# pnnl/nmrfit

Hardware: NVIDIA B200
Metric: voigt_objective_evals_per_s (higher is better)
Workload: dtype f64

## Files before the change

### include/nmrfit_b200.h

```cpp
#ifndef NMRFIT_B200_H
#define NMRFIT_B200_H

#ifdef __cplusplus
extern "C" {
#endif

#define NMRFIT_ABI_VERSION 2

#define NMRFIT_OK 0
#define NMRFIT_ERR_ARG (-1)
#define NMRFIT_ERR_CUDA (-2)
#define NMRFIT_ERR_STATE (-3)
#define NMRFIT_ERR_NOMEM (-4)

#define NMRFIT_FP64 0
#define NMRFIT_FP32 1

#define NMRFIT_ALGO_AUTO 0
#define NMRFIT_ALGO_GENERAL 1
#define NMRFIT_ALGO_UNIFORM 2

#define NMRFIT_REAL_ONLY 0
#define NMRFIT_IM_REFERENCE 1
#define NMRFIT_IM_SUM 2
// ... 31 lines not shown
#define NMRFIT_REFINE_MAX_ITER 3
#define NMRFIT_REFINE_NONFINITE 4

int nmrfit_ctx_refine(nmrfit_ctx* ctx, double* x_inout, const double* lb, const double* ub, int max_iter, double xtol,
                      double* f_out, int* passes_out, int* accepted_out, int* status_out, void* stream);

int nmrfit_ctx_set_algorithm(nmrfit_ctx* ctx, int algorithm);
int nmrfit_ctx_get_algorithm(nmrfit_ctx* ctx, int fit_im, int* algorithm);

int nmrfit_ctx_set_tuning(nmrfit_ctx* ctx, int threads, int points_per_thread, int exp_table_bits,
                          int particles_per_cta);
int nmrfit_ctx_get_tuning(nmrfit_ctx* ctx, int n_particles, int* threads, int* points_per_thread, int* exp_table_bits,
                          int* particles_per_cta, int* n_point_tiles);
int nmrfit_ctx_set_variant(nmrfit_ctx* ctx, int variant, int stages, int occupancy);
int nmrfit_ctx_get_variant(nmrfit_ctx* ctx, int n_particles, int* variant, int* stages);
int nmrfit_ctx_set_far_cells(nmrfit_ctx* ctx, int cells);

#define NMRFIT_FUSED_AUTO 0
#define NMRFIT_FUSED_OFF 1
#define NMRFIT_FUSED_REQUIRE 2
int nmrfit_ctx_set_fused(nmrfit_ctx* ctx, int mode);
int nmrfit_ctx_fused_launches(nmrfit_ctx* ctx, long long* launches);
int nmrfit_ctx_fused_timing(nmrfit_ctx* ctx, int enable, long long* cycles);

int nmrfit_ctx_profile(nmrfit_ctx* ctx, int enable);
int nmrfit_ctx_profile_read(nmrfit_ctx* ctx, double* total_ms, long long* launches);
int nmrfit_ctx_profile_read_split(nmrfit_ctx* ctx, double* prepare_ms, double* evaluate_ms, long long* launches);

int nmrfit_objective_batch(nmrfit_ctx* ctx, const double* x_dev, int n_particles, int fit_im, double* f_dev,
                           void* stream);
// ... 94 lines not shown
```

### nmrfit_b200/_cabi.py

```python
import ctypes
import os

import numpy as np

_HERE = os.path.dirname(os.path.abspath(__file__))
LIB_PATH = os.environ.get('NMRFIT_B200_LIB') or os.path.join(_HERE, 'csrc', 'libnmrfit_b200.so')

OK = 0
FP64, FP32 = 0, 1
REAL_ONLY, IM_REFERENCE, IM_SUM = 0, 1, 2
ALGO_AUTO, ALGO_GENERAL, ALGO_UNIFORM = 0, 1, 2
FUSED_AUTO, FUSED_OFF, FUSED_REQUIRE = 0, 1, 2
RUNNING, STOP_MINFUNC, STOP_MINSTEP, STOP_MAXITER, STOP_PEER_LOST = 0, 1, 2, 3, 4
REFINE_CONVERGED, REFINE_STALLED, REFINE_MAX_ITER, REFINE_NONFINITE = 1, 2, 3, 4

c_double_p = ctypes.POINTER(ctypes.c_double)
c_int_p = ctypes.POINTER(ctypes.c_int)


class NmrfitError(RuntimeError):

    def __init__(self, code, message):
        super().__init__('libnmrfit_b200 error %d: %s' % (code, message))
        self.code = code
# ... 15 lines not shown
    'nmrfit_device_count': (_i, [c_int_p]),
    'nmrfit_ctx_create': (_i, [ctypes.POINTER(_vp), _i, _i, _i, _i, _i]),
    'nmrfit_ctx_destroy': (None, [_vp]),
    'nmrfit_ctx_set_spectrum': (_i, [_vp, _i, _vp, _vp, _vp, _vp]),
    'nmrfit_ctx_set_spectra': (_i, [_vp, _i, _i, _vp, _vp, _vp, _vp]),
    'nmrfit_ctx_compute_weights': (_i, [_vp, _vp, _vp, _i, _i, _d, _vp, _vp]),
    'nmrfit_ctx_normal_equations': (_i, [_vp, _vp, _vp, _vp, _vp, _vp, _vp]),
    'nmrfit_normal_eq_plan': (_i, [_i, _i, c_int_p]),
    'nmrfit_ctx_refine': (_i, [_vp, _vp, _vp, _vp, _i, _d, _vp, _vp, _vp, _vp, _vp]),
    'nmrfit_ctx_set_algorithm': (_i, [_vp, _i]),
    'nmrfit_ctx_get_algorithm': (_i, [_vp, _i, c_int_p]),
    'nmrfit_ctx_set_tuning': (_i, [_vp, _i, _i, _i, _i]),
    'nmrfit_ctx_get_tuning': (_i, [_vp, _i, c_int_p, c_int_p, c_int_p, c_int_p, c_int_p]),
    'nmrfit_ctx_set_variant': (_i, [_vp, _i, _i, _i]),
    'nmrfit_ctx_get_variant': (_i, [_vp, _i, c_int_p, c_int_p]),
    'nmrfit_ctx_set_far_cells': (_i, [_vp, _i]),
    'nmrfit_ctx_set_fused': (_i, [_vp, _i]),
    'nmrfit_ctx_fused_launches': (_i, [_vp, ctypes.POINTER(ctypes.c_longlong)]),
    'nmrfit_ctx_fused_timing': (_i, [_vp, _i, _vp]),
    'nmrfit_ctx_profile': (_i, [_vp, _i]),
    'nmrfit_ctx_profile_read': (_i, [_vp, c_double_p, ctypes.POINTER(ctypes.c_longlong)]),
    'nmrfit_ctx_profile_read_split': (_i, [_vp, c_double_p, c_double_p, ctypes.POINTER(ctypes.c_longlong)]),
    'nmrfit_objective_batch': (_i, [_vp, _vp, _i, _i, _vp, _vp]),
    'nmrfit_objective_batch_host': (_i, [_vp, _vp, _i, _i, _vp]),
    'nmrfit_ctx_mt19937_shape': (_i, [_vp, ctypes.c_longlong]),
    'nmrfit_ctx_mt19937': (_i, [_vp, _vp, c_int_p, ctypes.c_longlong, ctypes.POINTER(_vp), ctypes.POINTER(_vp), _vp]),
    'nmrfit_pso_begin': (_i, [_vp, _vp, _vp, ctypes.POINTER(PsoOpts), _vp, _vp, _vp]),
    'nmrfit_pso_advance': (_i, [_vp, _vp, _vp, _vp]),
    'nmrfit_pso_step': (_i, [_vp, _vp, _vp, _vp]),
    'nmrfit_pso_peer_export': (_i, [_vp, _i, _i, _vp, ctypes.POINTER(_vp)]),
# ... 203 lines not shown
    def set_algorithm(self, algorithm=ALGO_AUTO):
        check(lib().nmrfit_ctx_set_algorithm(self._h, int(algorithm)))

    def get_algorithm(self, fit_im=REAL_ONLY):
        a = ctypes.c_int(0)
        check(lib().nmrfit_ctx_get_algorithm(self._h, int(fit_im), ctypes.byref(a)))
        return a.value

    def set_tuning(self, threads=0, points_per_thread=0, exp_table_bits=0, particles_per_cta=0):
        check(lib().nmrfit_ctx_set_tuning(self._h, threads, points_per_thread, exp_table_bits, particles_per_cta))

    def get_tuning(self, n_particles):
        vals = [ctypes.c_int(0) for _ in range(5)]
        check(lib().nmrfit_ctx_get_tuning(self._h, int(n_particles), *[ctypes.byref(v) for v in vals]))
        keys = ('threads', 'points_per_thread', 'exp_table_bits', 'particles_per_cta', 'n_point_tiles')
        return dict(zip(keys, (v.value for v in vals)))

    def set_variant(self, variant=-1, stages=0, occupancy=0):
        check(lib().nmrfit_ctx_set_variant(self._h, int(variant), int(stages), int(occupancy)))

    def set_far_cells(self, cells=0):
        check(lib().nmrfit_ctx_set_far_cells(self._h, int(cells)))

    def get_variant(self, n_particles):
        v, st = ctypes.c_int(0), ctypes.c_int(0)
        check(lib().nmrfit_ctx_get_variant(self._h, int(n_particles), ctypes.byref(v), ctypes.byref(st)))
        return v.value, st.value

    def set_fused(self, mode=FUSED_AUTO):
        check(lib().nmrfit_ctx_set_fused(self._h, int(mode)))

# ... 395 lines not shown
```

### nmrfit_b200/csrc/cabi.cu

```cuda
#include <cuda_runtime.h>
#include <algorithm>
#include <cmath>
#include <atomic>
#include <cstdio>
#include <cstring>
#include <memory>
#include <new>
#include <string>
#include <utility>
#include <vector>
#include "../../include/nmrfit_b200.h"
#include "nmrfit_internal.h"

namespace nmrfit {
std::atomic<long long> g_launches{0};
void count_launches(int n) { g_launches.fetch_add(n, std::memory_order_relaxed); }
}

using namespace nmrfit;

namespace {

thread_local std::string t_error;

// ... 62 lines not shown
}

}

constexpr int kShadowSpectra = 4;

struct nmrfit_ctx {
    int device = 0, B = 0, N = 0, P = 0, D = 0, precision = 0;
    DevBuf<double> spec;
    std::vector<char> spec_set;
    std::vector<std::vector<double>> shadow;
    DevBuf<double> grid_h;
    std::vector<char> uniform;
    int algorithm = NMRFIT_ALGO_AUTO;
    DevBuf<double> partials, x_stage, f_stage;
    DevBuf<double> prep_coef, prep_part, prep_far, prep_anchor;
    DevBuf<unsigned> prep_mask;
    ObjTune user_tune{0, 0, 0, 0, -1, 0, 0};
    bool swarm = false;
    SwarmState sw{};
    int maxiter = 0, kk = 0, generation = 0;
    DevBuf<double> sx, sv, sp, sfx, sfp, sg, sfg, sbx, sbf, slb, sub, srec, rnd_a, rnd_b;
    DevBuf<int> sstop, sit;
    DevBuf<double> frec_f, frec_x;
    DevBuf<unsigned> fbarrier;
    DevBuf<int> ferror;
    DevBuf<unsigned> mt_state;
    DevBuf<unsigned> mt_words;
    long long mt_elems = 0;
    DevBuf<double> mt_a[2], mt_b[2];
    DevBuf<unsigned> mt_state2, mt_words2;
// ... 63 lines not shown
    grid[0] = h;
    grid[1] = 2.220446049250313e-16 * big;
    return uni;
}

bool use_uniform(const nmrfit_ctx* c, int fit_im) {
    if (c->algorithm == NMRFIT_ALGO_GENERAL) return false;
    if (fit_im == NMRFIT_IM_SUM || (fit_im == NMRFIT_IM_REFERENCE && c->precision != NMRFIT_FP64)) return false;
    for (char u : c->uniform)
        if (!u) return false;
    return true;
}

int ctx_cells(const nmrfit_ctx* c, int r) { return c->far_cells ? c->far_cells : far_cells_per_region(c->N, r); }

ObjTune pick_tune(const nmrfit_ctx* c, int S, bool uni) {
    ObjTune t;
    if (uni) {
        if (c->N >= 2048) { t.threads = 256; t.r = 8; }
        else { t.threads = 128; t.r = 4; }
    } else {
        if (c->N >= 8192) { t.threads = 256; t.r = 4; }
        else if (c->N >= 1024) { t.threads = 128; t.r = 4; }
        else { t.threads = 128; t.r = 2; }
    }
    t.tb = 6;
    if (c->user_tune.threads) t.threads = c->user_tune.threads;
    if (c->user_tune.r) t.r = c->user_tune.r;
    if (c->user_tune.tb == -1) t.tb = 0;
    else if (c->user_tune.tb > 0) t.tb = c->user_tune.tb;
    int n_tiles = (c->N + t.threads * t.r - 1) / (t.threads * t.r);
    long long ctas1 = (long long)n_tiles * S * c->B;
    int sp = (int)std::max<long long>(1, std::min<long long>(16, ctas1 / (148 * 4)));
    sp = std::min(sp, std::max(1, S));
    if (c->user_tune.sp > 0) sp = std::min(c->user_tune.sp, std::max(1, S));
    t.sp = sp;
    t.variant = 0;
    t.stages = 0;
    t.occ = 3;
    const long long particle_tiles = (long long)((c->N + t.threads * t.r - 1) / (t.threads * t.r)) * S * c->B;
    const bool enough = particle_tiles >= 8192 || c->user_tune.variant == 1;
    if (uni && c->precision == NMRFIT_FP64 && c->user_tune.variant != 0 && t.tb == 6 && enough) {
        t.variant = 1;
        t.occ = c->user_tune.occ == 3 ? 3 : 2;
        const size_t budget = t.occ == 2 ? 115712 : 74 * 1024;
        const int cells = ctx_cells(c, t.r), per_warp = t.occ == 2 ? cells : 1;
        auto fit_sp = [&](int stg) {
            t.stages = stg;
            int spg = 0;
            for (int cand = 1; cand <= 16; ++cand) {
                t.sp = cand;
                if (objective_stream_smem_bytes(c->P, t, cells) <= budget && (cand < per_warp || cand % per_warp == 0))
                    spg = cand;
            }
            return spg;
        };
        int stg = c->user_tune.stages > 0 ? c->user_tune.stages : 3;
        int spg = fit_sp(stg);
        if (c->user_tune.stages == 0 && spg < 6) {
            const int spg2 = fit_sp(2);
            if (spg2 > spg) { stg = 2; spg = spg2; }
        }
        t.stages = stg;
        t.sp = std::max(1, spg);
        bool fits = true;
        if (c->user_tune.sp > 0) {
            t.sp = c->user_tune.sp;
            if (objective_stream_smem_bytes(c->P, t, ctx_cells(c, t.r)) > 200 * 1024 && c->user_tune.stages == 0) t.stages = 2;
            fits = objective_stream_smem_bytes(c->P, t, ctx_cells(c, t.r)) <= 200 * 1024;
        }
        if (fits) {
            t.sp = std::min(t.sp, std::max(1, S));
            return t;
        }
        t.variant = 0;
        t.stages = 0;
        t.occ = 3;
    }
    const bool f32 = c->precision == NMRFIT_FP32;
    auto uni_bytes = [&]() { return f32 ? objective_f32_smem_bytes(c->P, t) : objective_uniform_smem_bytes(c->P, t, ctx_cells(c, t.r)); };
    while (t.sp > 1 && (uni ? uni_bytes() : objective_smem_bytes(c->P, t, 2)) > 200 * 1024)
        t.sp /= 2;
    if (uni && c->user_tune.sp <= 0)
        while (t.sp > 4 && uni_bytes() > 74 * 1024) t.sp -= 1;
    return t;
}

int check_ctx(const nmrfit_ctx* c) {
    if (!c) return fail(NMRFIT_ERR_ARG, "ctx is NULL");
    return NMRFIT_OK;
}

// ... 12 lines not shown

struct ObjOut {
    int n_tiles = 0, nsum = 1, nw = 1;
};

int run_objective(nmrfit_ctx* c, const double* x_dev, int S, int fit_im, double* f_dev, cudaStream_t st,
                  const ObjIn& in = {}, ObjOut* out = nullptr) {
    for (int b = 0; b < c->B; ++b)
        if (!c->spec_set[b]) return fail(NMRFIT_ERR_STATE, "spectrum " + std::to_string(b) + " was never set");
    if (fit_im < 0 || fit_im > 2) return fail(NMRFIT_ERR_ARG, "fit_im must be 0, 1 or 2");
    const bool uni = use_uniform(c, fit_im);
    if (c->algorithm == NMRFIT_ALGO_UNIFORM && !uni)
        return fail(NMRFIT_ERR_STATE, "the uniform-axis kernel needs uniformly spaced w in every spectrum and fit_im off");
    if (c->precision == NMRFIT_FP32 && fit_im != NMRFIT_REAL_ONLY)
        return fail(NMRFIT_ERR_ARG, "fit_im is not available in FP32 mode (the Kramers-Kronig term runs in FP64 only)");
    ObjTune t = pick_tune(c, S, uni);
    if (uni && c->precision == NMRFIT_FP32 && t.r == 16) t.r = 8;
    if (uni ? (t.r != 4 && t.r != 8 && t.r != 16) : (t.r != 2 && t.r != 4 && t.r != 8))
        return fail(NMRFIT_ERR_ARG, uni ? "points_per_thread must be 4, 8 or 16 for the uniform-axis kernel"
                                        : "points_per_thread must be 2, 4 or 8 for the general kernel");
    int n_tiles = objective_tiles(c->N, t);
    const size_t part_per = (size_t)n_tiles * 2 * (t.variant == 1 ? t.threads / 32 : 1);
    CK(c->partials.reserve(std::max((size_t)c->B * S, in.slots_total) * part_per));
    ObjArgs a{};
    const int sub = (uni && c->precision == NMRFIT_FP64) ? ctx_cells(c, t.r) : 1;
    if (uni) {
        size_t nc, np, nf, na, nm;
        int pad = 0;
        objective_uniform_prep_sizes(c->N, c->P, t, sub, &nc, &np, &nf, &na, &nm, &pad);
        const size_t slots = std::max((size_t)c->B * S, in.slots_total) + pad;
        CK(c->prep_coef.reserve(slots * nc));
        CK(c->prep_part.reserve(slots * np));
        CK(c->prep_far.reserve(slots * nf));
        CK(c->prep_anchor.reserve(slots * na));
        CK(c->prep_mask.reserve(slots * nm));
        a.prep_coef = c->prep_coef.ptr + in.slot0 * nc; a.prep_part = c->prep_part.ptr + in.slot0 * np;
        a.prep_far = c->prep_far.ptr + in.slot0 * nf; a.prep_anchor = c->prep_anchor.ptr + in.slot0 * na;
        a.prep_mask = c->prep_mask.ptr + in.slot0 * nm;
    }
    a.spec = c->spec.ptr;
    a.x = x_dev;
    a.x_in = in.x_in;
    a.partials = c->partials.ptr + in.slot0 * part_per;
    a.frozen = in.frozen;
    a.grid_h = c->grid_h.ptr;
    a.N = c->N; a.P = c->P; a.S = S; a.kk = fit_im; a.sp = t.sp; a.sub = sub;
    cudaEvent_t ev0 = nullptr, evm = nullptr, ev1 = nullptr;
    if (c->profiling) {
        if (c->prof_used + 3 > c->prof_events.size()) {
            for (int k = 0; k < 3; ++k) {
                cudaEvent_t ev;
                CK(cudaEventCreate(&ev));
                c->prof_events.emplace_back(ev);
// ... 28 lines not shown

int stage(const double* src, size_t n, DevBuf<double>& buf, cudaStream_t st, const double** out) {
    if (!src) { *out = nullptr; return NMRFIT_OK; }
    if (is_device_pointer(src)) { *out = src; return NMRFIT_OK; }
    CK(buf.reserve(n));
    CK(cudaMemcpyAsync(buf.ptr, src, n * sizeof(double), cudaMemcpyHostToDevice, st));
    *out = buf.ptr;
    return NMRFIT_OK;
}

int fused_setup(nmrfit_ctx* c, int n_gen, const double* rp_d, const double* rg_d, FusedArgs* a, FusedPlan* plan) {
    plan->ok = false;
    if (c->fused_mode == NMRFIT_FUSED_OFF) return NMRFIT_OK;
    if (c->precision != NMRFIT_FP64 || c->kk != NMRFIT_REAL_ONLY || !use_uniform(c, NMRFIT_REAL_ONLY)) return NMRFIT_OK;
    const SwarmState& s = c->sw;
    ObjTune t = pick_tune(c, s.S, true);
    *a = FusedArgs{};
    a->s = s;
    a->spec = c->spec.ptr;
    a->grid_h = c->grid_h.ptr;
    a->rp = rp_d;
    a->rg = rg_d;
    a->N = c->N; a->P = c->P;
    a->n_vtiles = objective_tiles(c->N, t);
    a->vw = t.threads / 32;
    a->sub = ctx_cells(c, t.r);
    a->n_gen = n_gen;
    a->gen0 = c->generation + 1;
    a->maxiter = c->maxiter;
    cudaError_t e = swarm_fused_plan(*a, c->D, s.B, s.S, t, c->device, c->fused_mode == NMRFIT_FUSED_REQUIRE, plan);
    if (e != cudaSuccess) return fail_cuda(e, "fused swarm plan");
// ... 360 lines not shown
    c->user_tune.variant = variant;
    c->user_tune.stages = stages;
    c->user_tune.occ = occupancy;
    return NMRFIT_OK;
}

int nmrfit_ctx_set_far_cells(nmrfit_ctx* c, int cells) {
    if (int rc = check_ctx(c)) return rc;
    if (cells != 0 && cells != 1 && cells != 2 && cells != 4) return fail(NMRFIT_ERR_ARG, "cells must be 0 (auto), 1, 2 or 4");
    c->far_cells = cells;
    return NMRFIT_OK;
}

int nmrfit_ctx_get_variant(nmrfit_ctx* c, int S, int* variant, int* stages) {
    if (int rc = check_ctx(c)) return rc;
    ObjTune t = pick_tune(c, S < 1 ? 1 : S, use_uniform(c, NMRFIT_REAL_ONLY));
    if (variant) *variant = t.variant;
    if (stages) *stages = t.stages;
    return NMRFIT_OK;
}

int nmrfit_ctx_get_tuning(nmrfit_ctx* c, int S, int* threads, int* r, int* tb, int* sp, int* n_tiles) {
    if (int rc = check_ctx(c)) return rc;
    ObjTune t = pick_tune(c, S < 1 ? 1 : S, use_uniform(c, NMRFIT_REAL_ONLY));
    if (threads) *threads = t.threads;
    if (r) *r = t.r;
    if (tb) *tb = t.tb;
    if (sp) *sp = t.sp;
    if (n_tiles) *n_tiles = objective_tiles(c->N, t);
    return NMRFIT_OK;
}

int nmrfit_ctx_set_fused(nmrfit_ctx* c, int mode) {
    if (int rc = check_ctx(c)) return rc;
    if (mode != NMRFIT_FUSED_AUTO && mode != NMRFIT_FUSED_OFF && mode != NMRFIT_FUSED_REQUIRE)
        return fail(NMRFIT_ERR_ARG, "mode must be NMRFIT_FUSED_AUTO, _OFF or _REQUIRE");
    c->fused_mode = mode;
    return NMRFIT_OK;
}
// ... 948 lines not shown
```

### nmrfit_b200/csrc/nmrfit_internal.h

```cpp
#pragma once
#include <cuda_runtime.h>
#include <cstddef>
#include <cstdint>

#define NMRFIT_MAX_DEVICES 16

namespace nmrfit {

void count_launches(int n);

struct ObjArgs {
    const double* spec;
    const double* x;
    const double* x_in;
    double* partials;
    const int* frozen;
    const double* grid_h;
    double* prep_coef;
    double* prep_part;
    double* prep_far;
    double* prep_anchor;
    unsigned* prep_mask;
    int n_tiles, nw;
    int N, P, S;
    int kk;
    int sp;
    int tile_major;
    int stages, gpc, occ;
    int sub;
};

__host__ __device__ inline int far_cells_per_region(int N, int R) {
    const int target = N < 8192 ? 64 : (N < 32768 ? 128 : 256);
    int sub = 32 * R / target;
    return sub < 1 ? 1 : (sub > 4 ? 4 : sub);
}

struct ObjTune {
    int threads;
    int r;
    int tb;
    int sp;
    int variant;
    int stages;
    int occ;
};

int objective_tiles(int N, const ObjTune& t);
size_t objective_smem_bytes(int P, const ObjTune& t, int kk);
cudaError_t launch_objective(ObjArgs a, const ObjTune& t, int B, double* f, cudaStream_t st, cudaEvent_t ev0 = nullptr,
                             cudaEvent_t ev1 = nullptr, int* tiles_out = nullptr);

cudaError_t launch_objective_finalize(const double* partials, int n_tiles, int nsum, int N, int S, int B,
                                      const int* frozen, double* f, cudaStream_t st, int nw = 1);

size_t objective_uniform_smem_bytes(int P, const ObjTune& t, int sub = 1);
void objective_uniform_prep_sizes(int N, int P, const ObjTune& t, int sub, size_t* coef, size_t* part, size_t* far,
                                  size_t* anchor, size_t* mask_words, int* pad_particles);
struct SwarmState;
struct MoveArgs;
cudaError_t launch_objective_uniform(ObjArgs a, const ObjTune& t, int B, double* f, cudaStream_t st,
                                     cudaEvent_t ev0 = nullptr, cudaEvent_t ev1 = nullptr, const MoveArgs* mv = nullptr,
                                     int* tiles_out = nullptr, cudaEvent_t evm = nullptr, int* nw_out = nullptr);

cudaError_t launch_objective_prepare(ObjArgs& a, const ObjTune& t, int B, cudaStream_t st, const MoveArgs* mv = nullptr);

size_t objective_stream_smem_bytes(int P, const ObjTune& t, int sub);
cudaError_t launch_objective_stream(const ObjArgs& a, const ObjTune& t, int B, cudaStream_t st);

size_t objective_f32_smem_bytes(int P, const ObjTune& t);
cudaError_t launch_objective_f32(ObjArgs a, const ObjTune& t, int B, double* f, bool uniform, cudaStream_t st,
                                 cudaEvent_t ev0 = nullptr, cudaEvent_t ev1 = nullptr, int* tiles_out = nullptr);

// ... 131 lines not shown
```

### nmrfit_b200/csrc/objective_stream.cu

```cuda
#include <cuda_runtime.h>
#include <algorithm>
#include <cstdint>
#include "nmrfit_internal.h"
#include "nmrfit_math.cuh"
#include "uniform_common.cuh"
#include "uniform_eval.cuh"

namespace nmrfit {

namespace {

template <int TB> struct ExpTabS { static __device__ __forceinline__ const double* src() { return nullptr; } };
template <> struct ExpTabS<6> { static __device__ __forceinline__ const double* src() { return NMRFIT_EXP2_TAB6; } };

struct StreamSmem {
    int tab, uv, wt, wfirst, bars, tickets, slot0, slot, coef, part, far, anchor, mask, mw, total;
    __host__ __device__ StreamSmem(int spg, int stages, int P, int threads, int R, int TB, int sub) {
        const int nw = threads / 32;
        mw = (P + 31) / 32;
        int o = 0;
        tab = o;     o += TB ? (1 << TB) : 0;
        uv = o;      o += threads * R * 2;
        wt = o;      o += threads * R;
        wfirst = o;  o += threads;
        bars = o;    o += stages;
        tickets = o; o += (stages + 1) / 2 * 2;
        if (o & 1) ++o;
        slot0 = o;
        int q = 0;
        coef = q;    q += spg * P * 8;
        part = q;    q += spg * kPartDoubles;
        far = q;     q += spg * nw * sub * kFarPoly;
        anchor = q;  q += spg * nw * 2;
        mask = q;    q += ((spg * nw * mask_words_per_region(P, sub) + 3) / 4) * 2;
        slot = q;
        total = slot0 + stages * slot;
    }
};

__device__ __forceinline__ void fence_proxy_async_smem() { asm volatile("fence.proxy.async.shared::cta;" ::: "memory"); }

template <int THREADS, int R, int TB, int KK, int OCC, int SUB>
__global__ void __launch_bounds__(THREADS, (R <= 8 ? OCC * 256 : 512) / THREADS)
objective_stream_kernel(ObjArgs a) {
    constexpr int NSUM = KK ? 2 : 1;
    constexpr int NW = THREADS / 32;
    constexpr bool MULTI = SUB > 1 && !KK && OCC == 2;
    extern __shared__ __align__(16) double smem[];
    const int b = blockIdx.z;
    if (a.frozen && a.frozen[b]) return;
    const int tid = threadIdx.x, lane = tid & 31, warp = tid >> 5;
    const int P = a.P, N = a.N, D = 4 + 3 * P, SPG = a.sp, ST = a.stages;
    const int n_tiles = a.n_tiles, tile = blockIdx.y, NRP = n_tiles * NW;
    const StreamSmem L(SPG, ST, P, THREADS, R, TB, SUB);
    const int MW = L.mw;
    double* tab = smem + L.tab;
    double2* suv = reinterpret_cast<double2*>(smem + L.uv);
    double* swt = smem + L.wt;
    double* swf = smem + L.wfirst;
    uint64_t* bars = reinterpret_cast<uint64_t*>(smem + L.bars);
    int* tickets = reinterpret_cast<int*>(smem + L.tickets);
    double* slots = smem + L.slot0;

    const int n_groups = (a.S + SPG - 1) / SPG;
    const int g_lo = blockIdx.x * a.gpc, g_hi = min(n_groups, g_lo + a.gpc);
    const int my_groups = g_hi - g_lo;
    if (my_groups <= 0) return;

    const int tile0 = tile * (THREADS * R);
    const double* sw = a.spec + (size_t)b * 4 * N;
    const double h = a.grid_h[2 * b], w_ulp = a.grid_h[2 * b + 1];
    const size_t pb = (size_t)b * a.S;
    const size_t tb_ = ((size_t)b * n_tiles + tile) * a.S;

    const uint32_t b_coef = SPG * P * 8 * 8, b_part = SPG * kPartDoubles * 8, b_far = SPG * NW * SUB * kFarPoly * 8;
    const int MWR = mask_words_per_region(P, SUB);
    const uint32_t b_anchor = SPG * NW * 2 * 8, b_mask = SPG * NW * MWR * 4;
    auto fill = [&](int g) {
        const int sl = g % ST;
        double* dst = slots + (size_t)sl * L.slot;
        const size_t q0 = (size_t)(g_lo + g) * SPG;
        uint64_t* bar = bars + sl;
        mbar_expect_tx(bar, b_coef + b_part + b_far + b_anchor + b_mask);
        bulk_g2s(dst + L.coef, a.prep_coef + (pb + q0) * P * 8, b_coef, bar);
        bulk_g2s(dst + L.part, a.prep_part + (pb + q0) * kPartDoubles, b_part, bar);
        bulk_g2s(dst + L.far, a.prep_far + (tb_ + q0) * NW * SUB * kFarPoly, b_far, bar);
        bulk_g2s(dst + L.anchor, a.prep_anchor + (tb_ + q0) * NW * 2, b_anchor, bar);
        bulk_g2s(dst + L.mask, a.prep_mask + (tb_ + q0) * NW * MWR, b_mask, bar);
    };

    if (tid == 0) {
        for (int s = 0; s < ST; ++s) {
            mbar_init(bars + s, 1);
            tickets[s] = 0;
        }
        asm volatile("fence.mbarrier_init.release.cluster;" ::: "memory");
        for (int g = 0; g < min(ST, my_groups); ++g) fill(g);
    }
    for (int e = tid; e < THREADS * R; e += THREADS) {
        const int i = tile0 + e;
        const bool ok = i < N;
        const int t = e / R, j = e % R;
        const double wgt = ok ? sw[3 * N + i] : 0.0;
// ... 22 lines not shown
        const double* slot = slots + (size_t)sl * L.slot;
        const size_t q0 = (size_t)(g_lo + g) * SPG;
        const int nsp = min(SPG, a.S - (int)q0);
        const int rw = (warp + g) & (NW - 1);
        const int t = rw * 32 + lane;
        const int i_first = tile0 + t * R;
        const double w_first = swf[t];
        const double* cf = slot + L.coef;
        const double* pt = slot + L.part;
        const double* fc = slot + L.far + rw * SUB * kFarPoly;
        const double2* an = reinterpret_cast<const double2*>(slot + L.anchor) + rw;
        const unsigned* mk = reinterpret_cast<const unsigned*>(slot + L.mask) + rw * MWR;
        const double* xs = a.x + (pb + q0) * D;
        double* out = a.partials + (((pb + q0) * n_tiles + tile) * NW + rw) * NSUM;
        mbar_wait(bars + sl, phase);
        if constexpr (MULTI) {
            constexpr int LPC = 32 / SUB;
            const int q = lane / LPC;
            for (int sp0 = 0; sp0 < nsp; sp0 += SUB) {
                const int sp = min(sp0 + q, nsp - 1);
                const double ss = eval_region_multi<R, TB, SUB>(
                    cf + sp * s_coef, pt + sp * kPartDoubles, mk + sp * s_mask, fc + sp * s_far, an[sp * NW], MW, P, lane,
                    xi0, inv_H, suv, swt, swf, rw * 32, THREADS, tab, xs + (size_t)sp * D, sw + tile0, N - tile0, h, w_ulp);
                if ((lane & (LPC - 1)) == 0 && sp0 + q < nsp) out[sp * s_out] = ss;
            }
        } else for (int sp = 0; sp < nsp; ++sp) {
            double ssi = 0.0;
            const double ss = eval_region<R, TB, KK, false, SUB>(cf, pt, mk, fc, *an, MW, P, lane, lcell, w_first, xi0, inv_H, suv,
                                                            swt, t, THREADS, tab, xs, sw + i_first, N - i_first, h, w_ulp,
                                                            &ssi);
            if (lane == 0) {
// ... 8 lines not shown
            const int old = atomicAdd(tickets + sl, 1);
            if (old == NW - 1) {
                tickets[sl] = 0;
                __threadfence_block();
                if (g + ST < my_groups) {
                    fence_proxy_async_smem();
                    fill(g + ST);
                }
            }
        }
        if (++sl == ST) { sl = 0; phase ^= 1u; }
    }
    (void)NRP;
}

template <int THREADS, int R, int TB, int KK, int OCC, int SUB>
cudaError_t launch_sub(const ObjArgs& a, int B, cudaStream_t st) {
    static bool attr_set[NMRFIT_MAX_DEVICES] = {};
    StreamSmem L(a.sp, a.stages, a.P, THREADS, R, TB, a.sub);
    const size_t bytes = (size_t)L.total * sizeof(double);
    int dev = 0;
    cudaGetDevice(&dev);
    if (!attr_set[dev % NMRFIT_MAX_DEVICES]) {
        cudaError_t e = cudaFuncSetAttribute(objective_stream_kernel<THREADS, R, TB, KK, OCC, SUB>,
                                             cudaFuncAttributeMaxDynamicSharedMemorySize, 200 * 1024);
        if (e != cudaSuccess) return e;
        attr_set[dev % NMRFIT_MAX_DEVICES] = true;
    }
    const int n_groups = (a.S + a.sp - 1) / a.sp;
    dim3 grid((n_groups + a.gpc - 1) / a.gpc, a.n_tiles, B);
    objective_stream_kernel<THREADS, R, TB, KK, OCC, SUB><<<grid, THREADS, bytes, st>>>(a);
    return cudaGetLastError();
}

template <int THREADS, int R, int TB, int KK, int OCC>
cudaError_t launch_occ(const ObjArgs& a, int B, cudaStream_t st) {
    switch (a.sub) {
        case 1: return launch_sub<THREADS, R, TB, KK, OCC, 1>(a, B, st);
        case 2: return launch_sub<THREADS, R, TB, KK, OCC, 2>(a, B, st);
        case 4: return launch_sub<THREADS, R, TB, KK, OCC, 4>(a, B, st);
        default: return cudaErrorInvalidValue;
    }
}

template <int THREADS, int R, int TB, int KK>
cudaError_t launch_one(const ObjArgs& a, int B, cudaStream_t st) {
    return a.occ == 2 ? launch_occ<THREADS, R, TB, KK, 2>(a, B, st) : launch_occ<THREADS, R, TB, KK, 3>(a, B, st);
}

template <int THREADS, int R>
cudaError_t launch_tb(const ObjArgs& a, int tb, int B, cudaStream_t st) {
    switch (tb) {
        case 6: return a.kk ? launch_one<THREADS, R, 6, 1>(a, B, st) : launch_one<THREADS, R, 6, 0>(a, B, st);
        default: return cudaErrorInvalidValue;
    }
}

}

size_t objective_stream_smem_bytes(int P, const ObjTune& t, int sub) {
    return (size_t)StreamSmem(t.sp, t.stages, P, t.threads, t.r, t.tb, sub).total * sizeof(double);
}

cudaError_t launch_objective_stream(const ObjArgs& a, const ObjTune& t, int B, cudaStream_t st) {
    if (t.threads == 128 && t.r == 4) return launch_tb<128, 4>(a, t.tb, B, st);
    if (t.threads == 128 && t.r == 8) return launch_tb<128, 8>(a, t.tb, B, st);
    if (t.threads == 128 && t.r == 16) return launch_tb<128, 16>(a, t.tb, B, st);
    if (t.threads == 256 && t.r == 4) return launch_tb<256, 4>(a, t.tb, B, st);
    if (t.threads == 256 && t.r == 8) return launch_tb<256, 8>(a, t.tb, B, st);
    if (t.threads == 256 && t.r == 16) return launch_tb<256, 16>(a, t.tb, B, st);
    return cudaErrorInvalidValue;
}

}
```

### nmrfit_b200/csrc/objective_uniform.cu

```cuda
#include <cuda_runtime.h>
#include <algorithm>
#include <cstdint>
#include "nmrfit_internal.h"
#include "nmrfit_math.cuh"
#include "uniform_common.cuh"
#include "uniform_eval.cuh"
#include "swarm_common.cuh"

namespace nmrfit {

template <int TB> struct ExpTabU { static __device__ __forceinline__ const double* src() { return nullptr; } };
template <> struct ExpTabU<6> { static __device__ __forceinline__ const double* src() { return NMRFIT_EXP2_TAB6; } };
template <> struct ExpTabU<8> { static __device__ __forceinline__ const double* src() { return NMRFIT_EXP2_TAB8; } };
template <> struct ExpTabU<10> { static __device__ __forceinline__ const double* src() { return NMRFIT_EXP2_TAB10; } };


struct RegionDst {
    size_t base, tile_stride;
    int shift, mask;
    __device__ RegionDst(const ObjArgs& a, int b, int s, int NRP) {
        shift = a.nw == 8 ? 3 : 2;
        mask = a.nw - 1;
        if (a.tile_major) {
            base = ((size_t)b * a.n_tiles * a.S + s) * a.nw;
// ... 71 lines not shown
        } else {
            const RegionDst rd(a, b, s0 + g, NRP);
            dst = a.prep_anchor + rd.region(it - kTableItems) * 2;
        }
        *reinterpret_cast<double2*>(dst) = make_double2(cn, sn);
    }
    for (int e = nthreads - 1 - tid; e < ng * P; e += nthreads) {
        const int g = fast_div(e, P, inv_P), k = e - g * P;
        const double* xs = xsm + (size_t)g * D;
        prep_item_coef<R>(xs, k, h, w_ulp, cs + (size_t)g * P * 8, a.prep_coef + (ps0 + g) * P * 8,
                          farpk + (size_t)g * P * 4, sub, P, a.prep_part + (ps0 + g) * kPartDoubles);
    }
    __syncthreads();
    for (int e = tid; e < ng; e += nthreads)
        prep_item_exact_count(cs + (size_t)e * P * 8, P, a.prep_part + (ps0 + e) * kPartDoubles);
    const float inv_nc = 1.0f / (float)nc;
    const int sub_shift = sub == 4 ? 2 : sub == 2 ? 1 : 0;
    for (int base = tid & ~31; base < ng * nc; base += nthreads) {
        const int e = base + (tid & 31);
        const bool ok = e < ng * nc;
        const int g = ok ? fast_div(e, nc, inv_nc) : 0, cl = ok ? e - g * nc : 0;
        const int rl = cl >> sub_shift, ci = cl & (sub - 1);
        const RegionDst rd(a, b, s0 + g, NRP);
        const size_t rs = rd.region(rl);
        prep_item_cell<R>(ok, cs + (size_t)g * P * 8, farpk + (size_t)g * P * 4, sw, h, N, P, sub, (long long)cl * cell_pts, ci, nullptr,
                          a.prep_far + (rs * sub + ci) * kFarPoly, a.prep_mask + rs * MWR);
    }
}

struct UniSmem {
// ... 125 lines not shown
    return cudaGetLastError();
}

template <int THREADS, int R>
static cudaError_t launch_tb(const ObjArgs& a, int tb, int B, cudaStream_t st) {
    switch (tb) {
        case 0: return a.kk ? launch_one<THREADS, R, 0, 1>(a, B, st) : launch_one<THREADS, R, 0, 0>(a, B, st);
        case 6: return a.kk ? launch_one<THREADS, R, 6, 1>(a, B, st) : launch_one<THREADS, R, 6, 0>(a, B, st);
        case 8: return a.kk ? launch_one<THREADS, R, 8, 1>(a, B, st) : launch_one<THREADS, R, 8, 0>(a, B, st);
        case 10: return a.kk ? launch_one<THREADS, R, 10, 1>(a, B, st) : launch_one<THREADS, R, 10, 0>(a, B, st);
        default: return cudaErrorInvalidValue;
    }
}

void objective_uniform_prep_sizes(int N, int P, const ObjTune& t, int sub, size_t* coef, size_t* part, size_t* far,
                                  size_t* anchor, size_t* mask_words, int* pad_particles) {
    const size_t nrp = (size_t)objective_tiles(N, t) * (t.threads / 32);
    *coef = (size_t)P * 8;
    *part = kPartDoubles;
    *far = nrp * sub * kFarPoly;
    *anchor = nrp * 2;
    *mask_words = nrp * mask_words_per_region(P, sub);
    *pad_particles = kPadParticles;
}

size_t objective_uniform_smem_bytes(int P, const ObjTune& t, int sub) {
    return (size_t)UniSmem(t.sp, P, t.threads, t.r, t.tb, 2, sub).total * sizeof(double);
}

cudaError_t launch_objective_prepare(ObjArgs& a, const ObjTune& t, int B, cudaStream_t st, const MoveArgs* mv) {
    if (t.sp > kPadParticles) return cudaErrorInvalidValue;
    a.sp = t.sp;
    a.n_tiles = objective_tiles(a.N, t);
    a.nw = t.threads / 32;
    if (a.sub < 1) a.sub = 1;
    const int nc = a.n_tiles * a.nw * a.sub;
    const size_t per_particle = (size_t)(a.P * 12 + 4 + 3 * a.P) * sizeof(double);
    int G = std::max(1, std::min(16, std::min(a.S, 4 * kPrepThreads / nc)));
    while (G > 1 && G * per_particle > 40 * 1024) --G;
    int pthreads = nc >= 128 ? 128 : kPrepThreads;
    if (nc >= 128) G = 1;
    const long long want_ctas = 2 * 148;
    if ((long long)a.S * B / G < want_ctas) {
        G = (int)std::max<long long>(1, std::min<long long>(G, (long long)a.S * B / want_ctas));
        if (G == 1) pthreads = 128;
    }
    dim3 pgrid((a.S + G - 1) / G, B);
    const size_t bytes = G * per_particle;
    const MoveArgs none{};
    if (mv) {
        if (t.r == 4) objective_prepare_kernel<4, true><<<pgrid, pthreads, bytes, st>>>(a, *mv, G);
        else if (t.r == 8) objective_prepare_kernel<8, true><<<pgrid, pthreads, bytes, st>>>(a, *mv, G);
        else if (t.r == 16) objective_prepare_kernel<16, true><<<pgrid, pthreads, bytes, st>>>(a, *mv, G);
// ... 56 lines not shown
```

Before: 76.05 million.

## Build far-field cells inside the stream kernel instead of the prepare pass

Adds a CELLS variant of the streaming objective kernel. The prepare kernel now writes only a compact per-particle packed far-field array, and each warp rebuilds its far-field polynomials and masks in shared-memory scratch just before evaluating. This removes the large per-region far/mask global buffers and their bulk copies, trading them for extra per-warp compute and per-warp scratch shared memory, which can lower particles per group. It is enabled automatically for real-only FP64 uniform runs with four cells per region and R<=8.

```diff
diff --git a/include/nmrfit_b200.h b/include/nmrfit_b200.h
--- a/include/nmrfit_b200.h
+++ b/include/nmrfit_b200.h
@@ -69,6 +69,7 @@
                           int* particles_per_cta, int* n_point_tiles);
 int nmrfit_ctx_set_variant(nmrfit_ctx* ctx, int variant, int stages, int occupancy);
 int nmrfit_ctx_get_variant(nmrfit_ctx* ctx, int n_particles, int* variant, int* stages);
+int nmrfit_ctx_get_stream_cells(nmrfit_ctx* ctx, int n_particles, int* in_kernel);
 int nmrfit_ctx_set_far_cells(nmrfit_ctx* ctx, int cells);
 
 #define NMRFIT_FUSED_AUTO 0
diff --git a/nmrfit_b200/_cabi.py b/nmrfit_b200/_cabi.py
--- a/nmrfit_b200/_cabi.py
+++ b/nmrfit_b200/_cabi.py
@@ -53,6 +53,7 @@
     'nmrfit_ctx_get_tuning': (_i, [_vp, _i, c_int_p, c_int_p, c_int_p, c_int_p, c_int_p]),
     'nmrfit_ctx_set_variant': (_i, [_vp, _i, _i, _i]),
     'nmrfit_ctx_get_variant': (_i, [_vp, _i, c_int_p, c_int_p]),
+    'nmrfit_ctx_get_stream_cells': (_i, [_vp, _i, c_int_p]),
     'nmrfit_ctx_set_far_cells': (_i, [_vp, _i]),
     'nmrfit_ctx_set_fused': (_i, [_vp, _i]),
     'nmrfit_ctx_fused_launches': (_i, [_vp, ctypes.POINTER(ctypes.c_longlong)]),
@@ -286,7 +287,11 @@
         vals = [ctypes.c_int(0) for _ in range(5)]
         check(lib().nmrfit_ctx_get_tuning(self._h, int(n_particles), *[ctypes.byref(v) for v in vals]))
         keys = ('threads', 'points_per_thread', 'exp_table_bits', 'particles_per_cta', 'n_point_tiles')
-        return dict(zip(keys, (v.value for v in vals)))
+        out = dict(zip(keys, (v.value for v in vals)))
+        cells = ctypes.c_int(0)
+        check(lib().nmrfit_ctx_get_stream_cells(self._h, int(n_particles), ctypes.byref(cells)))
+        out['stream_cells_in_kernel'] = bool(cells.value)
+        return out
 
     def set_variant(self, variant=-1, stages=0, occupancy=0):
         check(lib().nmrfit_ctx_set_variant(self._h, int(variant), int(stages), int(occupancy)))
diff --git a/nmrfit_b200/csrc/cabi.cu b/nmrfit_b200/csrc/cabi.cu
--- a/nmrfit_b200/csrc/cabi.cu
+++ b/nmrfit_b200/csrc/cabi.cu
@@ -100,7 +100,7 @@
     std::vector<char> uniform;
     int algorithm = NMRFIT_ALGO_AUTO;
     DevBuf<double> partials, x_stage, f_stage;
-    DevBuf<double> prep_coef, prep_part, prep_far, prep_anchor;
+    DevBuf<double> prep_coef, prep_part, prep_far, prep_anchor, prep_farpk;
     DevBuf<unsigned> prep_mask;
     ObjTune user_tune{0, 0, 0, 0, -1, 0, 0};
     bool swarm = false;
@@ -194,8 +194,8 @@
 
 int ctx_cells(const nmrfit_ctx* c, int r) { return c->far_cells ? c->far_cells : far_cells_per_region(c->N, r); }
 
-ObjTune pick_tune(const nmrfit_ctx* c, int S, bool uni) {
-    ObjTune t;
+ObjTune pick_tune(const nmrfit_ctx* c, int S, bool uni, bool real_only) {
+    ObjTune t{};
     if (uni) {
         if (c->N >= 2048) { t.threads = 256; t.r = 8; }
         else { t.threads = 128; t.r = 4; }
@@ -225,22 +225,33 @@
         t.occ = c->user_tune.occ == 3 ? 3 : 2;
         const size_t budget = t.occ == 2 ? 115712 : 74 * 1024;
         const int cells = ctx_cells(c, t.r), per_warp = t.occ == 2 ? cells : 1;
+        const int per_round = 32 / cells;
         auto fit_sp = [&](int stg) {
             t.stages = stg;
             int spg = 0;
             for (int cand = 1; cand <= 16; ++cand) {
                 t.sp = cand;
-                if (objective_stream_smem_bytes(c->P, t, cells) <= budget && (cand < per_warp || cand % per_warp == 0))
-                    spg = cand;
+                const bool whole = t.cells ? cand % per_round == 0 : (cand < per_warp || cand % per_warp == 0);
+                if (objective_stream_smem_bytes(c->P, t, cells) <= budget && whole) spg = cand;
             }
             return spg;
         };
-        int stg = c->user_tune.stages > 0 ? c->user_tune.stages : 3;
-        int spg = fit_sp(stg);
-        if (c->user_tune.stages == 0 && spg < 6) {
-            const int spg2 = fit_sp(2);
-            if (spg2 > spg) { stg = 2; spg = spg2; }
+        auto fit_stages = [&](int* spg) {
+            int stg = c->user_tune.stages > 0 ? c->user_tune.stages : 3;
+            *spg = fit_sp(stg);
+            if (c->user_tune.stages == 0 && *spg < 6) {
+                const int spg2 = fit_sp(2);
+                if (spg2 > *spg) { stg = 2; *spg = spg2; }
+            }
+            return stg;
+        };
+        int spg = 0, stg = 0;
+        t.cells = real_only && t.occ == 2 && cells == 4 && t.r <= 8 && c->user_tune.sp % per_round == 0;
+        if (t.cells) {
+            stg = fit_stages(&spg);
+            if (spg == 0) t.cells = 0;
         }
+        if (!t.cells) stg = fit_stages(&spg);
         t.stages = stg;
         t.sp = std::max(1, spg);
         bool fits = true;
@@ -256,6 +267,7 @@
         t.variant = 0;
         t.stages = 0;
         t.occ = 3;
+        t.cells = 0;
     }
     const bool f32 = c->precision == NMRFIT_FP32;
     auto uni_bytes = [&]() { return f32 ? objective_f32_smem_bytes(c->P, t) : objective_uniform_smem_bytes(c->P, t, ctx_cells(c, t.r)); };
@@ -298,7 +310,7 @@
         return fail(NMRFIT_ERR_STATE, "the uniform-axis kernel needs uniformly spaced w in every spectrum and fit_im off");
     if (c->precision == NMRFIT_FP32 && fit_im != NMRFIT_REAL_ONLY)
         return fail(NMRFIT_ERR_ARG, "fit_im is not available in FP32 mode (the Kramers-Kronig term runs in FP64 only)");
-    ObjTune t = pick_tune(c, S, uni);
+    ObjTune t = pick_tune(c, S, uni, fit_im == NMRFIT_REAL_ONLY);
     if (uni && c->precision == NMRFIT_FP32 && t.r == 16) t.r = 8;
     if (uni ? (t.r != 4 && t.r != 8 && t.r != 16) : (t.r != 2 && t.r != 4 && t.r != 8))
         return fail(NMRFIT_ERR_ARG, uni ? "points_per_thread must be 4, 8 or 16 for the uniform-axis kernel"
@@ -309,18 +321,22 @@
     ObjArgs a{};
     const int sub = (uni && c->precision == NMRFIT_FP64) ? ctx_cells(c, t.r) : 1;
     if (uni) {
-        size_t nc, np, nf, na, nm;
+        size_t nc, np, nf, na, nm, nk;
         int pad = 0;
-        objective_uniform_prep_sizes(c->N, c->P, t, sub, &nc, &np, &nf, &na, &nm, &pad);
+        objective_uniform_prep_sizes(c->N, c->P, t, sub, &nc, &np, &nf, &na, &nm, &nk, &pad);
         const size_t slots = std::max((size_t)c->B * S, in.slots_total) + pad;
         CK(c->prep_coef.reserve(slots * nc));
         CK(c->prep_part.reserve(slots * np));
-        CK(c->prep_far.reserve(slots * nf));
         CK(c->prep_anchor.reserve(slots * na));
-        CK(c->prep_mask.reserve(slots * nm));
+        CK(c->prep_farpk.reserve(slots * nk));
         a.prep_coef = c->prep_coef.ptr + in.slot0 * nc; a.prep_part = c->prep_part.ptr + in.slot0 * np;
-        a.prep_far = c->prep_far.ptr + in.slot0 * nf; a.prep_anchor = c->prep_anchor.ptr + in.slot0 * na;
-        a.prep_mask = c->prep_mask.ptr + in.slot0 * nm;
+        a.prep_anchor = c->prep_anchor.ptr + in.slot0 * na; a.prep_farpk = c->prep_farpk.ptr + in.slot0 * nk;
+        if (!t.cells) {
+            CK(c->prep_far.reserve(slots * nf));
+            CK(c->prep_mask.reserve(slots * nm));
+            a.prep_far = c->prep_far.ptr + in.slot0 * nf;
+            a.prep_mask = c->prep_mask.ptr + in.slot0 * nm;
+        }
     }
     a.spec = c->spec.ptr;
     a.x = x_dev;
@@ -379,7 +395,7 @@
     if (c->fused_mode == NMRFIT_FUSED_OFF) return NMRFIT_OK;
     if (c->precision != NMRFIT_FP64 || c->kk != NMRFIT_REAL_ONLY || !use_uniform(c, NMRFIT_REAL_ONLY)) return NMRFIT_OK;
     const SwarmState& s = c->sw;
-    ObjTune t = pick_tune(c, s.S, true);
+    ObjTune t = pick_tune(c, s.S, true, true);
     *a = FusedArgs{};
     a->s = s;
     a->spec = c->spec.ptr;
@@ -770,15 +786,22 @@
 
 int nmrfit_ctx_get_variant(nmrfit_ctx* c, int S, int* variant, int* stages) {
     if (int rc = check_ctx(c)) return rc;
-    ObjTune t = pick_tune(c, S < 1 ? 1 : S, use_uniform(c, NMRFIT_REAL_ONLY));
+    ObjTune t = pick_tune(c, S < 1 ? 1 : S, use_uniform(c, NMRFIT_REAL_ONLY), true);
     if (variant) *variant = t.variant;
     if (stages) *stages = t.stages;
     return NMRFIT_OK;
 }
 
+int nmrfit_ctx_get_stream_cells(nmrfit_ctx* c, int S, int* in_kernel) {
+    if (int rc = check_ctx(c)) return rc;
+    ObjTune t = pick_tune(c, S < 1 ? 1 : S, use_uniform(c, NMRFIT_REAL_ONLY), true);
+    if (in_kernel) *in_kernel = t.variant == 1 && t.cells;
+    return NMRFIT_OK;
+}
+
 int nmrfit_ctx_get_tuning(nmrfit_ctx* c, int S, int* threads, int* r, int* tb, int* sp, int* n_tiles) {
     if (int rc = check_ctx(c)) return rc;
-    ObjTune t = pick_tune(c, S < 1 ? 1 : S, use_uniform(c, NMRFIT_REAL_ONLY));
+    ObjTune t = pick_tune(c, S < 1 ? 1 : S, use_uniform(c, NMRFIT_REAL_ONLY), true);
     if (threads) *threads = t.threads;
     if (r) *r = t.r;
     if (tb) *tb = t.tb;
diff --git a/nmrfit_b200/csrc/nmrfit_internal.h b/nmrfit_b200/csrc/nmrfit_internal.h
--- a/nmrfit_b200/csrc/nmrfit_internal.h
+++ b/nmrfit_b200/csrc/nmrfit_internal.h
@@ -21,6 +21,8 @@
     double* prep_far;
     double* prep_anchor;
     unsigned* prep_mask;
+    double* prep_farpk;
+    int cells;
     int n_tiles, nw;
     int N, P, S;
     int kk;
@@ -44,6 +46,7 @@
     int variant;
     int stages;
     int occ;
+    int cells;
 };
 
 int objective_tiles(int N, const ObjTune& t);
@@ -56,7 +59,7 @@
 
 size_t objective_uniform_smem_bytes(int P, const ObjTune& t, int sub = 1);
 void objective_uniform_prep_sizes(int N, int P, const ObjTune& t, int sub, size_t* coef, size_t* part, size_t* far,
-                                  size_t* anchor, size_t* mask_words, int* pad_particles);
+                                  size_t* anchor, size_t* mask_words, size_t* farpk, int* pad_particles);
 struct SwarmState;
 struct MoveArgs;
 cudaError_t launch_objective_uniform(ObjArgs a, const ObjTune& t, int B, double* f, cudaStream_t st,
diff --git a/nmrfit_b200/csrc/objective_stream.cu b/nmrfit_b200/csrc/objective_stream.cu
--- a/nmrfit_b200/csrc/objective_stream.cu
+++ b/nmrfit_b200/csrc/objective_stream.cu
@@ -14,8 +14,9 @@
 template <> struct ExpTabS<6> { static __device__ __forceinline__ const double* src() { return NMRFIT_EXP2_TAB6; } };
 
 struct StreamSmem {
-    int tab, uv, wt, wfirst, bars, tickets, slot0, slot, coef, part, far, anchor, mask, mw, total;
-    __host__ __device__ StreamSmem(int spg, int stages, int P, int threads, int R, int TB, int sub) {
+    int tab, uv, wt, wfirst, bars, tickets, slot0, slot, coef, part, far, anchor, mask, farpk, mw, scratch, scr_far,
+        scr_warp, total;
+    __host__ __device__ StreamSmem(int spg, int stages, int P, int threads, int R, int TB, int sub, bool cells) {
         const int nw = threads / 32;
         mw = (P + 31) / 32;
         int o = 0;
@@ -30,29 +31,34 @@
         int q = 0;
         coef = q;    q += spg * P * 8;
         part = q;    q += spg * kPartDoubles;
-        far = q;     q += spg * nw * sub * kFarPoly;
+        far = q;     q += cells ? 0 : spg * nw * sub * kFarPoly;
         anchor = q;  q += spg * nw * 2;
-        mask = q;    q += ((spg * nw * mask_words_per_region(P, sub) + 3) / 4) * 2;
+        mask = q;    q += cells ? 0 : ((spg * nw * mask_words_per_region(P, sub) + 3) / 4) * 2;
+        farpk = q;   q += cells ? spg * P * 4 : 0;
         slot = q;
-        total = slot0 + stages * slot;
+        scratch = slot0 + stages * slot;
+        scr_far = 32 * kFarPoly;
+        scr_warp = cells ? scr_far + ((32 / sub * mask_words_per_region(P, sub) + 3) / 4) * 2 : 0;
+        total = scratch + nw * scr_warp;
     }
 };
 
 __device__ __forceinline__ void fence_proxy_async_smem() { asm volatile("fence.proxy.async.shared::cta;" ::: "memory"); }
 
-template <int THREADS, int R, int TB, int KK, int OCC, int SUB>
+template <int THREADS, int R, int TB, int KK, int OCC, int SUB, bool CELLS>
 __global__ void __launch_bounds__(THREADS, (R <= 8 ? OCC * 256 : 512) / THREADS)
 objective_stream_kernel(ObjArgs a) {
     constexpr int NSUM = KK ? 2 : 1;
     constexpr int NW = THREADS / 32;
     constexpr bool MULTI = SUB > 1 && !KK && OCC == 2;
+    static_assert((MULTI && SUB == 4 && R <= 8) || !CELLS, "in-kernel far-field cells: four cells per region, real part");
     extern __shared__ __align__(16) double smem[];
     const int b = blockIdx.z;
     if (a.frozen && a.frozen[b]) return;
     const int tid = threadIdx.x, lane = tid & 31, warp = tid >> 5;
     const int P = a.P, N = a.N, D = 4 + 3 * P, SPG = a.sp, ST = a.stages;
     const int n_tiles = a.n_tiles, tile = blockIdx.y, NRP = n_tiles * NW;
-    const StreamSmem L(SPG, ST, P, THREADS, R, TB, SUB);
+    const StreamSmem L(SPG, ST, P, THREADS, R, TB, SUB, CELLS);
     const int MW = L.mw;
     double* tab = smem + L.tab;
     double2* suv = reinterpret_cast<double2*>(smem + L.uv);
@@ -75,18 +81,22 @@
 
     const uint32_t b_coef = SPG * P * 8 * 8, b_part = SPG * kPartDoubles * 8, b_far = SPG * NW * SUB * kFarPoly * 8;
     const int MWR = mask_words_per_region(P, SUB);
-    const uint32_t b_anchor = SPG * NW * 2 * 8, b_mask = SPG * NW * MWR * 4;
+    const uint32_t b_anchor = SPG * NW * 2 * 8, b_mask = SPG * NW * MWR * 4, b_farpk = SPG * P * 4 * 8;
     auto fill = [&](int g) {
         const int sl = g % ST;
         double* dst = slots + (size_t)sl * L.slot;
         const size_t q0 = (size_t)(g_lo + g) * SPG;
         uint64_t* bar = bars + sl;
-        mbar_expect_tx(bar, b_coef + b_part + b_far + b_anchor + b_mask);
+        mbar_expect_tx(bar, b_coef + b_part + b_anchor + (CELLS ? b_farpk : b_far + b_mask));
         bulk_g2s(dst + L.coef, a.prep_coef + (pb + q0) * P * 8, b_coef, bar);
         bulk_g2s(dst + L.part, a.prep_part + (pb + q0) * kPartDoubles, b_part, bar);
-        bulk_g2s(dst + L.far, a.prep_far + (tb_ + q0) * NW * SUB * kFarPoly, b_far, bar);
         bulk_g2s(dst + L.anchor, a.prep_anchor + (tb_ + q0) * NW * 2, b_anchor, bar);
-        bulk_g2s(dst + L.mask, a.prep_mask + (tb_ + q0) * NW * MWR, b_mask, bar);
+        if (CELLS) {
+            bulk_g2s(dst + L.farpk, a.prep_farpk + (pb + q0) * P * 4, b_farpk, bar);
+        } else {
+            bulk_g2s(dst + L.far, a.prep_far + (tb_ + q0) * NW * SUB * kFarPoly, b_far, bar);
+            bulk_g2s(dst + L.mask, a.prep_mask + (tb_ + q0) * NW * MWR, b_mask, bar);
+        }
     };
 
     if (tid == 0) {
@@ -139,7 +149,30 @@
         const double* xs = a.x + (pb + q0) * D;
         double* out = a.partials + (((pb + q0) * n_tiles + tile) * NW + rw) * NSUM;
         mbar_wait(bars + sl, phase);
-        if constexpr (MULTI) {
+        if constexpr (CELLS) {
+            constexpr int LPC = 32 / SUB, PPR = 32 / SUB;
+            const int q = lane / LPC;
+            double* scr = smem + L.scratch + warp * L.scr_warp;
+            unsigned* smk = reinterpret_cast<unsigned*>(scr + L.scr_far);
+            const double* fpk = slot + L.farpk;
+            const long long ic = (long long)tile0 + rw * 32 * R + (lane % SUB) * (32 * R / SUB);
+            for (int r0 = 0; r0 < nsp; r0 += PPR) {
+                const int jp = lane / SUB, sb = r0 + jp;
+                prep_item_cell<R>(sb < nsp, cf + sb * s_coef, fpk + sb * P * 4, sw, h, N, P, SUB, ic, lane % SUB, nullptr,
+                                  scr + lane * kFarPoly, smk + jp * MWR);
+                __syncwarp();
+                const int rn = min(PPR, nsp - r0);
+                for (int sp0 = 0; sp0 < rn; sp0 += SUB) {
+                    const int j = min(sp0 + q, rn - 1), sp = r0 + j;
+                    const double ss = eval_region_multi<R, TB, SUB>(
+                        cf + sp * s_coef, pt + sp * kPartDoubles, smk + j * MWR, scr + j * SUB * kFarPoly, an[sp * NW], MW, P,
+                        lane, xi0, inv_H, suv, swt, swf, rw * 32, THREADS, tab, xs + (size_t)sp * D, sw + tile0, N - tile0, h,
+                        w_ulp);
+                    if ((lane & (LPC - 1)) == 0 && sp0 + q < rn) out[sp * s_out] = ss;
+                }
+                __syncwarp();
+            }
+        } else if constexpr (MULTI) {
             constexpr int LPC = 32 / SUB;
             const int q = lane / LPC;
             for (int sp0 = 0; sp0 < nsp; sp0 += SUB) {
@@ -178,23 +211,33 @@
     (void)NRP;
 }
 
-template <int THREADS, int R, int TB, int KK, int OCC, int SUB>
-cudaError_t launch_sub(const ObjArgs& a, int B, cudaStream_t st) {
+template <int THREADS, int R, int TB, int KK, int OCC, int SUB, bool CELLS>
+cudaError_t launch_cells(const ObjArgs& a, int B, cudaStream_t st) {
     static bool attr_set[NMRFIT_MAX_DEVICES] = {};
-    StreamSmem L(a.sp, a.stages, a.P, THREADS, R, TB, a.sub);
+    StreamSmem L(a.sp, a.stages, a.P, THREADS, R, TB, a.sub, CELLS);
     const size_t bytes = (size_t)L.total * sizeof(double);
     int dev = 0;
     cudaGetDevice(&dev);
     if (!attr_set[dev % NMRFIT_MAX_DEVICES]) {
-        cudaError_t e = cudaFuncSetAttribute(objective_stream_kernel<THREADS, R, TB, KK, OCC, SUB>,
+        cudaError_t e = cudaFuncSetAttribute(objective_stream_kernel<THREADS, R, TB, KK, OCC, SUB, CELLS>,
                                              cudaFuncAttributeMaxDynamicSharedMemorySize, 200 * 1024);
         if (e != cudaSuccess) return e;
         attr_set[dev % NMRFIT_MAX_DEVICES] = true;
     }
     const int n_groups = (a.S + a.sp - 1) / a.sp;
     dim3 grid((n_groups + a.gpc - 1) / a.gpc, a.n_tiles, B);
-    objective_stream_kernel<THREADS, R, TB, KK, OCC, SUB><<<grid, THREADS, bytes, st>>>(a);
+    objective_stream_kernel<THREADS, R, TB, KK, OCC, SUB, CELLS><<<grid, THREADS, bytes, st>>>(a);
     return cudaGetLastError();
+}
+
+template <int THREADS, int R, int TB, int KK, int OCC, int SUB>
+cudaError_t launch_sub(const ObjArgs& a, int B, cudaStream_t st) {
+    if constexpr (SUB == 4 && !KK && OCC == 2 && R <= 8) {
+        if (a.cells) return launch_cells<THREADS, R, TB, KK, OCC, SUB, true>(a, B, st);
+    } else {
+        if (a.cells) return cudaErrorInvalidValue;
+    }
+    return launch_cells<THREADS, R, TB, KK, OCC, SUB, false>(a, B, st);
 }
 
 template <int THREADS, int R, int TB, int KK, int OCC>
@@ -223,7 +266,7 @@
 }
 
 size_t objective_stream_smem_bytes(int P, const ObjTune& t, int sub) {
-    return (size_t)StreamSmem(t.sp, t.stages, P, t.threads, t.r, t.tb, sub).total * sizeof(double);
+    return (size_t)StreamSmem(t.sp, t.stages, P, t.threads, t.r, t.tb, sub, t.cells != 0).total * sizeof(double);
 }
 
 cudaError_t launch_objective_stream(const ObjArgs& a, const ObjTune& t, int B, cudaStream_t st) {
diff --git a/nmrfit_b200/csrc/objective_uniform.cu b/nmrfit_b200/csrc/objective_uniform.cu
--- a/nmrfit_b200/csrc/objective_uniform.cu
+++ b/nmrfit_b200/csrc/objective_uniform.cu
@@ -109,6 +109,10 @@
     __syncthreads();
     for (int e = tid; e < ng; e += nthreads)
         prep_item_exact_count(cs + (size_t)e * P * 8, P, a.prep_part + (ps0 + e) * kPartDoubles);
+    if (a.cells) {
+        for (int e = tid; e < ng * P * 4; e += nthreads) a.prep_farpk[ps0 * P * 4 + e] = farpk[e];
+        return;
+    }
     const float inv_nc = 1.0f / (float)nc;
     const int sub_shift = sub == 4 ? 2 : sub == 2 ? 1 : 0;
     for (int base = tid & ~31; base < ng * nc; base += nthreads) {
@@ -264,13 +268,14 @@
 }
 
 void objective_uniform_prep_sizes(int N, int P, const ObjTune& t, int sub, size_t* coef, size_t* part, size_t* far,
-                                  size_t* anchor, size_t* mask_words, int* pad_particles) {
+                                  size_t* anchor, size_t* mask_words, size_t* farpk, int* pad_particles) {
     const size_t nrp = (size_t)objective_tiles(N, t) * (t.threads / 32);
     *coef = (size_t)P * 8;
     *part = kPartDoubles;
     *far = nrp * sub * kFarPoly;
     *anchor = nrp * 2;
     *mask_words = nrp * mask_words_per_region(P, sub);
+    *farpk = (size_t)P * 4;
     *pad_particles = kPadParticles;
 }
 
@@ -284,9 +289,10 @@
     a.n_tiles = objective_tiles(a.N, t);
     a.nw = t.threads / 32;
     if (a.sub < 1) a.sub = 1;
-    const int nc = a.n_tiles * a.nw * a.sub;
+    a.cells = t.variant == 1 && t.cells;
+    const int nc = a.cells ? 0 : a.n_tiles * a.nw * a.sub;
     const size_t per_particle = (size_t)(a.P * 12 + 4 + 3 * a.P) * sizeof(double);
-    int G = std::max(1, std::min(16, std::min(a.S, 4 * kPrepThreads / nc)));
+    int G = std::max(1, std::min(16, nc ? std::min(a.S, 4 * kPrepThreads / nc) : a.S));
     while (G > 1 && G * per_particle > 40 * 1024) --G;
     int pthreads = nc >= 128 ? 128 : kPrepThreads;
     if (nc >= 128) G = 1;
```

After: 77.55 million, median of 6. 2.0% higher.
